# facebookresearch/NasRec

Hardware: AMD Instinct MI355X
Metric: supernet samples/sec at batch 256 (Criteo-shape), 1/2/4/8 MI355X (higher is better)
Workload: dtype f32

## Files before the change

### include/nasrec_hip.h

```cpp
#ifndef NASREC_HIP_H
#define NASREC_HIP_H

#include <stdint.h>

#ifdef __cplusplus
extern "C" {
#endif

#define NASREC_MAX_SEGS 8
#define NASREC_MAX_TABLES 32
#define NASREC_EMB_DIM 16
#define NASREC_MHA_PARAMS 1696
#define NASREC_MHA_SAVED 36

enum {
  NASREC_AM_KC = 0,
  NASREC_AM_RC = 1,
  NASREC_AM_TOKR = 2,
  NASREC_AM_TOKK = 3
};
enum { NASREC_CM_PLAIN = 0,
       NASREC_CM_TOKJ = 1    };
enum { NASREC_ACT_NONE = 0, NASREC_ACT_RELU = 1, NASREC_ACT_SILU = 2, NASREC_ACT_SIGMOID = 3 };

// ... 591 lines not shown
int nasrec_graph_destroy(void* graph);

int nasrec_gemm(void* stream, const nasrec_gemm_desc_t* d);
int nasrec_embedding_gather(void* stream, const nasrec_embed_desc_t* d);
int nasrec_embedding_dedup(void* stream, const nasrec_emb_dedup_desc_t* d);
int nasrec_dot_tri(void* stream, const nasrec_dot_tri_desc_t* d);
int nasrec_fm(void* stream, const nasrec_fm_desc_t* d);
int nasrec_mha_ffn(void* stream, const nasrec_mha_desc_t* d);
int nasrec_layernorm(void* stream, const nasrec_layernorm_desc_t* d);
int nasrec_final_logit(void* stream, const nasrec_final_desc_t* d);
int nasrec_bce_logits(void* stream, const nasrec_bce_desc_t* d);
int nasrec_adagrad_dense(void* stream, const nasrec_adagrad_dense_desc_t* d);
int nasrec_adagrad_rows(void* stream, const nasrec_adagrad_rows_desc_t* d);
int nasrec_opt_reduce(void* stream, const nasrec_opt_reduce_desc_t* d);
int nasrec_opt_apply(void* stream, const nasrec_opt_apply_desc_t* d);
int nasrec_dedup_ids(void* stream, const nasrec_dedup_ids_desc_t* d);
int nasrec_opt_reduce2(void* stream, const nasrec_opt_reduce2_desc_t* d);
int nasrec_final_fused(void* stream, const nasrec_final_desc_t* d);
int nasrec_weight_decay(void* stream, const nasrec_weight_decay_desc_t* d);
int nasrec_opt_moments(void* stream, const nasrec_opt_moments_desc_t* d);
int nasrec_last_layer_step(void* stream, const nasrec_last_layer_step_desc_t* d);
int nasrec_roc_auc(void* stream, const nasrec_roc_auc_desc_t* d);
int64_t nasrec_roc_auc_workspace_bytes(int64_t n);
int nasrec_worklist(void* stream, const nasrec_worklist_desc_t* d);

enum {
  NASREC_GEMM_ROUTE_GENERAL = 0,
  NASREC_GEMM_ROUTE_KSLICE = 1,
  NASREC_GEMM_ROUTE_SKINNY_N = 2,
  NASREC_GEMM_ROUTE_TINYK = 3,
  NASREC_GEMM_ROUTE_TOKEN_LINEAR = 4,
  NASREC_GEMM_ROUTE_TOKEN_DW = 5,
  NASREC_GEMM_ROUTE_FAST = 6,
  NASREC_GEMM_ROUTE_BAD_NSEG = -1,
  NASREC_GEMM_ROUTE_BAD_BINDING = -2,
  NASREC_GEMM_ROUTE_BAD_BALANCED = -3
};
int nasrec_gemm_route(const nasrec_gemm_desc_t* d, unsigned* eligible_mask);

int nasrec_alloc_uncached(int64_t bytes, void** out);
int nasrec_free_uncached(void* p);

int nasrec_event_create(void** ev);
int nasrec_event_record(void* ev, void* stream);
int nasrec_event_elapsed_ms(void* start, void* stop, float* ms);
int nasrec_event_destroy(void* ev);

enum { NASREC_TSV_OK = 0, NASREC_TSV_NEEDS_PYTHON = 1, NASREC_TSV_BAD_COLUMNS = 2 };
int64_t nasrec_tsv_parse(const char* buf, int64_t len, int32_t Fd, int32_t Fs, const int64_t* table_rows, int64_t max_rows,
                         int64_t* label, int64_t* dense, int64_t* cat, int64_t* consumed, int32_t* status);

const char* nasrec_last_error(void);
int nasrec_abi_version(void);
int nasrec_desc_sizes(int32_t* out, int n);

#ifdef __cplusplus
}
#endif
#endif
```

### nasrec_amd/_lib.py

```python
import ctypes as C
import os

import torch

_HERE = os.path.dirname(os.path.abspath(__file__))
LIB_PATH = os.environ.get("NASREC_HIP_LIB") or os.path.join(_HERE, "lib", "libnasrec_hip.so")

MAX_SEGS = 8
MAX_TABLES = 32
EMB_DIM = 16
MHA_PARAMS = 1696
MHA_SAVED = 36
REDUCE_MAX_DST = 48

AM_KC, AM_RC, AM_TOKR, AM_TOKK = 0, 1, 2, 3
CM_PLAIN, CM_TOKJ = 0, 1
ACT_NONE, ACT_RELU, ACT_SILU, ACT_SIGMOID = 0, 1, 2, 3
TSV_OK, TSV_NEEDS_PYTHON, TSV_BAD_COLUMNS = 0, 1, 2
ACT_BY_NAME = {"identity": ACT_NONE, "relu": ACT_RELU, "silu": ACT_SILU}

(OP_GEMM, OP_EMBED_GATHER, OP_DOT_TRI_FWD, OP_DOT_TRI_BWD, OP_FM_FWD, OP_FM_BWD, OP_MHA_FWD, OP_MHA_BWD, OP_REDUCE_ROWS,
 OP_COPY_SEGS, OP_GATE_BWD, OP_ROWSUM, OP_FINAL_FWD, OP_BCE, OP_FINAL_BWD, OP_EMB_DEDUP, OP_SUMSQ, OP_CLIP_COEF,
 OP_ADAGRAD_DENSE, OP_ADAGRAD_ROWS, OP_MEMSET, OP_LAYERNORM_FWD, OP_LAYERNORM_BWD, OP_ADD_SEGS, OP_SCALE,
 OP_ACT_BWD, OP_STAGE_INPUTS, OP_OPT_REDUCE, OP_OPT_APPLY, OP_WORKLIST, OP_CONST_I64, OP_SPLITK_EPILOGUES, OP_DEDUP_IDS,
# ... 84 lines not shown
                ("dlogits_out", vp), ("nsplit", i32), ("dseg_done", i32), ("tok_stride", i32 * MAX_SEGS)]


class BceDesc(C.Structure):
    _fields_ = [("kind", i32), ("B", i32), ("grad_scale", f32), ("_pad", i32), ("logits", vp), ("y", vp), ("loss", vp),
                ("dlogits", vp)]


class SumsqDesc(C.Structure):
    _fields_ = [("kind", i32), ("nblocks", i32), ("n", i64), ("x", vp), ("partial", vp), ("chunks", vp), ("nchunks", i64)]


class ClipCoefDesc(C.Structure):
    _fields_ = [("kind", i32), ("n_a", i32), ("n_b", i32), ("max_norm", f32), ("partial_a", vp), ("partial_b", vp), ("out", vp)]


class AdagradDenseDesc(C.Structure):
    _fields_ = [("kind", i32), ("eps", f32), ("n", i64), ("p", vp), ("g", vp), ("state", vp), ("lr", vp), ("coef", vp),
                ("chunks", vp), ("nchunks", i64)]


class AdagradRowsDesc(C.Structure):
    _fields_ = [("kind", i32), ("B", i32), ("Fs", i32), ("eps", f32), ("idx", vp), ("leader", vp), ("gsum", vp),
                ("table", vp * MAX_TABLES), ("state", vp * MAX_TABLES), ("lr", vp), ("coef", vp), ("rows", i64 * MAX_TABLES),
                ("rank_B", i32), ("_pad", i32), ("rank_stride", i64)]


class MemsetDesc(C.Structure):
    _fields_ = [("kind", i32), ("_pad", i32), ("bytes", i64), ("ptr", vp), ("chunks", vp), ("nchunks", i64)]


SPLITK_BALANCED = -1
(GEMM_ROUTE_GENERAL, GEMM_ROUTE_KSLICE, GEMM_ROUTE_SKINNY_N, GEMM_ROUTE_TINYK, GEMM_ROUTE_TOKEN_LINEAR, GEMM_ROUTE_TOKEN_DW,
 GEMM_ROUTE_FAST) = range(7)
GEMM_ROUTE_BAD_NSEG, GEMM_ROUTE_BAD_BINDING, GEMM_ROUTE_BAD_BALANCED = -1, -2, -3
SK_WORKSPACE_FLOATS = 512 * 3 * 128 * 128
CHUNK_ELEMS = 65536
CONST_I64_MAX = 448


class ConstI64Desc(C.Structure):
    _fields_ = [("kind", i32), ("n", i32), ("dst", vp), ("vals", i64 * CONST_I64_MAX)]


class LayerNormDesc(C.Structure):
    _fields_ = [("kind", i32), ("mode", i32), ("R", i32), ("D", i32), ("ldx", i32), ("ldy", i32), ("act", i32),
                ("dims_in_use", i32), ("accumulate", i32), ("eps", f32), ("x", vp), ("w", vp), ("b", vp), ("y", vp), ("stats", vp),
                ("dy", vp), ("dx", vp), ("dwb_partial", vp), ("nblk", i32), ("_pad", i32)]


class ScaleDesc(C.Structure):
    _fields_ = [("kind", i32), ("_pad", i32), ("n", i64), ("s", f32), ("_pad2", i32), ("x", vp), ("y", vp)]


class ActBwdDesc(C.Structure):
    _fields_ = [("kind", i32), ("mode", i32), ("R", i32), ("D", i32), ("ld_dy", i32), ("ld_z", i32), ("ld_dz", i32), ("act", i32),
                ("dims_in_use", i32), ("dy", vp), ("z", vp), ("dz", vp)]


DEDUP_IDS_MAX_B = 2048


class DedupIdsDesc(C.Structure):
    _fields_ = [("kind", i32), ("B", i32), ("Fs", i32), ("cap", i32), ("idx", vp), ("leader", vp), ("order", vp), ("lists", vp), ("counts", vp),
                ("heads", vp)]


# ... 167 lines not shown
```

### nasrec_amd/csrc/gemm.hip

```cpp
#include "gemm_tile.h"
#include "gemm_ring.h"

template <int AM, int BMODE, int CM, int NT, int TK, int TBM, int TBN>
__global__ __launch_bounds__(NT) void gemm_kernel(const nasrec_gemm_desc_t d, int Mmax, int Nmax) {
  gemm_tile<AM, BMODE, CM, NT, TK, TBM, TBN>(d, Mmax, Nmax, blockIdx.x, blockIdx.y, blockIdx.z);
}

#ifndef GEMM_RING
#define GEMM_RING 4
#endif
template <int AM, int BMODE, int CM, int NT, int TK, int TBM, int TBN, bool AUX>
__global__ __launch_bounds__(NT) void gemm_ring_kernel(const nasrec_gemm_desc_t d, int Mmax, int Nmax) {
  gemm_tile_ring<AM, BMODE, CM, NT, TK, TBM, TBN, AUX, AUX ? 2 : GEMM_RING>(d, Mmax, Nmax, blockIdx.x, blockIdx.y, blockIdx.z);
}

template <int CM>
__global__ __launch_bounds__(256) void gemm_splitk_epilogue(const nasrec_gemm_desc_t d, int Mmax, int Nmax) {
  splitk_second_pass<CM>(d, Mmax, Nmax, blockIdx.z, (long)blockIdx.x * 256 + threadIdx.x);
}

struct EpiGeom {
  int first[NASREC_EPILOGUES_MAX + 1];
  int per[NASREC_EPILOGUES_MAX];
  int Mmax[NASREC_EPILOGUES_MAX], Nmax[NASREC_EPILOGUES_MAX];
// ... 74 lines not shown
    } else if (deep) {
      launch_ring<AM, BMODE, CM, GEMM_MID_NT, GEMM_TK_DEEP, 64, 64>(st, d, Mmax, Nmax, zdim);
    } else {
      launch_ring<AM, BMODE, CM, GEMM_MID_NT, 32, 64, 64>(st, d, Mmax, Nmax, zdim);
    }
  } else if (Nmax >= Mmax) {
    if (deep) launch_ring<AM, BMODE, CM, 256, GEMM_TK_DEEP, 64, 16>(st, d, Mmax, Nmax, zdim);
    else launch_ring<AM, BMODE, CM, 256, 32, 64, 16>(st, d, Mmax, Nmax, zdim);
  } else {
    if (deep) launch_ring<AM, BMODE, CM, 256, GEMM_TK_DEEP, 16, 64>(st, d, Mmax, Nmax, zdim);
    else launch_ring<AM, BMODE, CM, 256, 32, 16, 64>(st, d, Mmax, Nmax, zdim);
  }
}

static constexpr int binding_key(int am, int bm, int cm) { return am * 100 + bm * 10 + cm; }

int nasrec_gemm_route(const nasrec_gemm_desc_t* d, unsigned* eligible_mask) {
  if (eligible_mask) *eligible_mask = 0;
  if (d->nseg < 1 || d->nseg > NASREC_MAX_SEGS) return NASREC_GEMM_ROUTE_BAD_NSEG;
  switch (binding_key(d->amode, d->bmode, d->cmode)) {
    case binding_key(NASREC_AM_KC, NASREC_AM_KC, NASREC_CM_PLAIN):
    case binding_key(NASREC_AM_KC, NASREC_AM_RC, NASREC_CM_PLAIN):
    case binding_key(NASREC_AM_RC, NASREC_AM_RC, NASREC_CM_PLAIN):
    case binding_key(NASREC_AM_KC, NASREC_AM_TOKR, NASREC_CM_TOKJ):
    case binding_key(NASREC_AM_RC, NASREC_AM_TOKR, NASREC_CM_TOKJ):
    case binding_key(NASREC_AM_TOKK, NASREC_AM_TOKK, NASREC_CM_PLAIN):
      break;
    default:
      return NASREC_GEMM_ROUTE_BAD_BINDING;
  }
  static const struct { int family; bool (*takes)(const nasrec_gemm_desc_t*); } ladder[] = {
    {NASREC_GEMM_ROUTE_TOKEN_LINEAR, token_linear_eligible},
    {NASREC_GEMM_ROUTE_KSLICE, gemm_kslice_eligible},
    {NASREC_GEMM_ROUTE_SKINNY_N, gemm_skinny_n_eligible},
    {NASREC_GEMM_ROUTE_TINYK, gemm_tinyk_eligible},
    {NASREC_GEMM_ROUTE_TOKEN_DW, token_dw_eligible},
    {NASREC_GEMM_ROUTE_FAST, gemm_fast_eligible},
  };
  const bool balanced = d->splitk == NASREC_SPLITK_BALANCED;
  int route = balanced ? NASREC_GEMM_ROUTE_BAD_BALANCED : NASREC_GEMM_ROUTE_GENERAL;
  unsigned mask = balanced ? 0u : 1u << NASREC_GEMM_ROUTE_GENERAL;
  bool taken = false;
  for (const auto& f : ladder) {
    if (!f.takes(d)) continue;
    mask |= 1u << f.family;
    if (!taken) route = f.family;
    taken = true;
    if (!eligible_mask) break;
  }
  if (eligible_mask) *eligible_mask = mask;
  return route;
}

int launch_gemm(hipStream_t st, const nasrec_gemm_desc_t* d) {
  const int route = nasrec_gemm_route(d, nullptr);
  if (route == NASREC_GEMM_ROUTE_BAD_NSEG) return nasrec_set_error(-2, "gemm: nseg=%d out of range", d->nseg);
  if (route == NASREC_GEMM_ROUTE_BAD_BINDING)
    return nasrec_set_error(-2, "gemm: unsupported operand binding a=%d b=%d c=%d", d->amode, d->bmode, d->cmode);
  int Mmax = 0, Nmax = 0;
  const int nprob = d->zmode ? d->nseg : 1;
  for (int q = 0; q < nprob; ++q) {
    if (d->seg[q].M > Mmax) Mmax = d->seg[q].M;
    if (d->seg[q].N > Nmax) Nmax = d->seg[q].N;
  }
  if (Mmax <= 0 || Nmax <= 0) return 0;
  const int S = d->splitk > 1 ? d->splitk : 1;
  if (S > 1 && d->workspace == nullptr) return nasrec_set_error(-3, "gemm: splitk=%d needs a workspace", S);
  switch (route) {
    case NASREC_GEMM_ROUTE_TOKEN_LINEAR: return launch_token_linear(st, d);
    case NASREC_GEMM_ROUTE_KSLICE: return launch_gemm_kslice(st, d);
    case NASREC_GEMM_ROUTE_SKINNY_N: return launch_gemm_skinny_n(st, d);
    case NASREC_GEMM_ROUTE_TINYK: return launch_gemm_tinyk(st, d);
    case NASREC_GEMM_ROUTE_BAD_BALANCED:
      return nasrec_set_error(-2, "gemm: the balanced schedule exists for throughput-regime launches only (the planner asks nasrec_gemm_route)");
    case NASREC_GEMM_ROUTE_TOKEN_DW: launch_token_dw(st, d, Mmax, Nmax); break;
    case NASREC_GEMM_ROUTE_FAST: {
      const int rc = launch_gemm_fast(st, d, Mmax, Nmax, nprob * S);
      if (rc) return rc;
      break;
    }
    default:
      switch (binding_key(d->amode, d->bmode, d->cmode)) {
        case binding_key(NASREC_AM_KC, NASREC_AM_KC, NASREC_CM_PLAIN): launch_general_t<NASREC_AM_KC, NASREC_AM_KC, NASREC_CM_PLAIN>(st, d, Mmax, Nmax, nprob, S); break;
        case binding_key(NASREC_AM_KC, NASREC_AM_RC, NASREC_CM_PLAIN): launch_general_t<NASREC_AM_KC, NASREC_AM_RC, NASREC_CM_PLAIN>(st, d, Mmax, Nmax, nprob, S); break;
        case binding_key(NASREC_AM_RC, NASREC_AM_RC, NASREC_CM_PLAIN): launch_general_t<NASREC_AM_RC, NASREC_AM_RC, NASREC_CM_PLAIN>(st, d, Mmax, Nmax, nprob, S); break;
        case binding_key(NASREC_AM_KC, NASREC_AM_TOKR, NASREC_CM_TOKJ): launch_general_t<NASREC_AM_KC, NASREC_AM_TOKR, NASREC_CM_TOKJ>(st, d, Mmax, Nmax, nprob, S); break;
        case binding_key(NASREC_AM_RC, NASREC_AM_TOKR, NASREC_CM_TOKJ): launch_general_t<NASREC_AM_RC, NASREC_AM_TOKR, NASREC_CM_TOKJ>(st, d, Mmax, Nmax, nprob, S); break;
        default: launch_general_t<NASREC_AM_TOKK, NASREC_AM_TOKK, NASREC_CM_PLAIN>(st, d, Mmax, Nmax, nprob, S); break;
      }
  }
  if (S > 1 && !d->defer_second_pass) {
    const dim3 g2((unsigned)(((long)Mmax * Nmax + 255) / 256), 1, nprob);
    if (d->cmode == NASREC_CM_PLAIN) hipLaunchKernelGGL((gemm_splitk_epilogue<NASREC_CM_PLAIN>), g2, dim3(256), 0, st, *d, Mmax, Nmax);
    else hipLaunchKernelGGL((gemm_splitk_epilogue<NASREC_CM_TOKJ>), g2, dim3(256), 0, st, *d, Mmax, Nmax);
  }
  return nasrec_check_launch("gemm");
}
```

### nasrec_amd/csrc/gemm_tile.h

```cpp
#pragma once
#include "common.h"

#ifndef GEMM_TK_DEEP
#define GEMM_TK_DEEP 64
#endif
#ifndef GEMM_XCD_REMAP
#define GEMM_XCD_REMAP 0
#endif
#ifndef GEMM_ZBATCH_TILE32
#define GEMM_ZBATCH_TILE32 1
#endif
#ifndef GEMM_BIG_NT
#define GEMM_BIG_NT 256
#endif
#ifndef GEMM_BIG_TK
#define GEMM_BIG_TK 32
#endif
#ifndef GEMM_MID_NT
#define GEMM_MID_NT 1024
#endif
#ifndef GEMM_SKINNY_BELOW
#define GEMM_SKINNY_BELOW 128
#endif
#ifndef NASREC_GEMM_FAST_MIN_TILES
#define NASREC_GEMM_FAST_MIN_TILES 120
#endif
bool gemm_fast_eligible(const nasrec_gemm_desc_t* d);
int launch_gemm_fast(hipStream_t st, const nasrec_gemm_desc_t* d, int Mmax, int Nmax, int zdim);
bool gemm_kslice_eligible(const nasrec_gemm_desc_t* d);
int launch_gemm_kslice(hipStream_t st, const nasrec_gemm_desc_t* d);
bool gemm_skinny_n_eligible(const nasrec_gemm_desc_t* d);
int launch_gemm_skinny_n(hipStream_t st, const nasrec_gemm_desc_t* d);
bool gemm_tinyk_eligible(const nasrec_gemm_desc_t* d);
int launch_gemm_tinyk(hipStream_t st, const nasrec_gemm_desc_t* d);
bool token_linear_eligible(const nasrec_gemm_desc_t* d);
int launch_token_linear(hipStream_t st, const nasrec_gemm_desc_t* d);
bool token_dw_eligible(const nasrec_gemm_desc_t* d);
int launch_token_dw(hipStream_t st, const nasrec_gemm_desc_t* d, int Mmax, int Nmax);

template <int MODE, int NT, int TK, int R>
__device__ __forceinline__ void stage_coords(int tid, int it, int& rr, int& kk) {
  if (MODE == NASREC_AM_KC || MODE == NASREC_AM_TOKK) {
    kk = tid & (TK - 1);
    rr = tid / TK + (NT / TK) * it;
  } else {
    rr = tid & (R - 1);
    kk = tid / R + (NT / R) * it;
  }
}

__device__ __forceinline__ float mul_lookup(const nasrec_gemm_desc_t& d, int i, int j) {
  for (int q = 0; q < d.mul_nseg; ++q) {
    int jj = j - d.mul_off[q];
    if (jj >= 0 && jj < d.mul_width[q]) return d.mul_ptr[q] ? d.mul_ptr[q][(long)i * d.mul_ld[q] + jj] : 0.f;
  }
  return 0.f;
}

__device__ __forceinline__ int seg_ld(const nasrec_gemm_desc_t& d, int sq, int which) {
  return which ? d.seg[sq].ldb : d.seg[sq].lda;
}

template <int CM>
// ... 397 lines not shown
```

### nasrec_amd/csrc/worklist.hip

```cpp
#include <stdlib.h>
#include <string.h>

#include <vector>

#include "worklist_body.h"

static int wl_gemm_geometry(const nasrec_gemm_desc_t* g, nasrec_wl_item_t& it, int blob_left) {
  if (g->nseg < 1 || g->nseg > NASREC_MAX_SEGS) return nasrec_set_error(-2, "worklist: gemm nseg=%d", g->nseg);
  const int need = (int)offsetof(nasrec_gemm_desc_t, seg) + g->nseg * (int)sizeof(nasrec_gemm_seg_t);
  if (need > blob_left) return nasrec_set_error(-2, "worklist: truncated gemm descriptor (%d bytes) runs past the blob", need);
  const int nprob = g->zmode ? g->nseg : 1;
  const int S = g->splitk > 1 ? g->splitk : 1;
  if (g->splitk == NASREC_SPLITK_BALANCED) return nasrec_set_error(-2, "worklist: the balanced schedule is a throughput-regime launch");
  if ((it.part == 0) != (S == 1)) return nasrec_set_error(-2, "worklist: gemm part %d with splitk %d", it.part, g->splitk);
  if (S > 1 && !g->workspace) return nasrec_set_error(-3, "worklist: splitk=%d needs a workspace", S);
  int Mmax = 0, Nmax = 0, Kmax = 0;
  long wgs = 0;
  bool aux = false, uniform = true;
  for (int q = 0; q < nprob; ++q) {
    Mmax = g->seg[q].M > Mmax ? g->seg[q].M : Mmax;
    Nmax = g->seg[q].N > Nmax ? g->seg[q].N : Nmax;
    wgs += (long)((g->seg[q].M + 63) / 64) * ((g->seg[q].N + 63) / 64) * S;
  }
  for (int q = 0; q < g->nseg; ++q) {
    const nasrec_gemm_seg_t& s = g->seg[q];
    if (s.A && s.K > Kmax) Kmax = s.K;
    aux = aux || s.Aaux || s.Baux;
    if (!g->zmode && (s.ones_col != g->seg[0].ones_col || s.Mvalid != g->seg[0].Mvalid)) uniform = false;
    if (!g->zmode && s.A && ((s.Aaux != nullptr) != (g->seg[0].Aaux != nullptr) || (s.Baux != nullptr) != (g->seg[0].Baux != nullptr))) uniform = false;
  }
  if (!uniform) return nasrec_set_error(-2, "worklist: k-segments that disagree on row predicates / mask operands take the plain template");
  {
    const bool kca = g->amode == NASREC_AM_KC || g->amode == NASREC_AM_TOKK, kcb = g->bmode == NASREC_AM_KC || g->bmode == NASREC_AM_TOKK;
    if (!kca && kcb) return nasrec_set_error(-2, "worklist: operand binding a=%d b=%d has no body", g->amode, g->bmode);
  }
  if (Mmax <= 0 || Nmax <= 0) {
    it.nblk = 0;
    return 0;
  }
  if (it.part == 2) {
    const int per = (int)(((long)Mmax * Nmax + 255) / 256);
    it.geom[0] = per;
    it.nblk = per * nprob;
    return 0;
  }
  static const bool dense_body = getenv("NASREC_WL_DENSE_BODY") == nullptr || atoi(getenv("NASREC_WL_DENSE_BODY")) != 0;
  if (dense_body && it.part == 0 && !g->zmode && !aux && g->amode == NASREC_AM_KC && g->bmode == NASREC_AM_KC && g->cmode == NASREC_CM_PLAIN) {
    bool plain = true;
    int steps = 0;
    for (int q = 0; q < g->nseg; ++q) {
      const nasrec_gemm_seg_t& s = g->seg[q];
      plain = plain && !s.ones_col && !(s.Mvalid > 0 && s.Mvalid < Mmax);
      plain = plain && (long)Mmax * s.lda + s.K < (1L << 29) && (long)Nmax * s.ldb + s.K < (1L << 29);
      steps += (s.A && s.K > 0) ? (s.K + 15) >> 4 : 1;
    }
    if (plain && steps <= 2 * WL_DENSE_STEPS && (Mmax + 15) / 16 < 0x10000) {
      it.geom[0] = (Nmax + 15) / 16;
      it.geom[1] = (Mmax + 15) / 16 | (((steps + WL_DENSE_STEPS - 1) / WL_DENSE_STEPS) << 16);
      it.geom[2] = WL_TOKS | (3 << 2);
      it.nblk = (it.geom[0] * ((Mmax + 15) / 16) + 3) / 4;
      return 0;
    }
  }
  bool aux_b = false;
  for (int q = 0; q < g->nseg; ++q) aux_b = aux_b || g->seg[q].Baux;
  if (dense_body && it.part == 0 && g->zmode && !aux_b && g->amode == NASREC_AM_KC && g->bmode == NASREC_AM_RC && g->cmode == NASREC_CM_PLAIN) {
    bool plain = true;
    int TU = 0;
    for (int q = 0; q < g->nseg; ++q) {
      const nasrec_gemm_seg_t& s = g->seg[q];
      plain = plain && !s.ones_col && !(s.Mvalid > 0 && s.Mvalid < s.M) && s.K <= 16 * WL_DENSE_STEPS && s.M > 0 && s.N > 0;
      plain = plain && (long)s.M * s.lda + s.K < (1L << 29) && (long)s.K * s.ldb + s.N < (1L << 29);
      TU += ((s.M + 15) / 16) * ((s.N + 15) / 16);
    }
    if (plain && TU > 0) {
      it.geom[0] = TU;
      it.geom[1] = 0;
      it.geom[2] = WL_TOKS | (3 << 2);
// ... 224 lines not shown
  out->_pad = 0;
  out->dev = reinterpret_cast<const nasrec_worklist_desc_t*>(dev_buf);
  return 0;
}

int launch_worklist_dev(hipStream_t st, const nasrec_worklist_dev_desc_t* d) {
  if (!d->dev) return nasrec_set_error(-2, "worklist (device-resident): not prepared");
  if (d->total_blocks < 1) return 0;
  const unsigned* pf = d->pf;
  const unsigned* pm = d->pm;
  if (d->big) {
    hipLaunchKernelGGL(worklist_dev_kernel<true>, dim3((unsigned)d->total_blocks), dim3(256), sizeof(float) * WL_LDS_BIG_FLOATS, st, pf[0], pf[1], pf[2], pf[3],
                       pf[4], pf[5], pm[0], pm[1], pm[2], pm[3], pm[4], pm[5], d->dev);
  } else {
    hipLaunchKernelGGL(worklist_dev_kernel<false>, dim3((unsigned)d->total_blocks), dim3(256), sizeof(float) * WL_LDS_FLOATS, st, pf[0], pf[1], pf[2], pf[3],
                       pf[4], pf[5], pm[0], pm[1], pm[2], pm[3], pm[4], pm[5], d->dev);
  }
  return nasrec_check_launch("worklist (device-resident)");
}

#define PS_SPIN_BUDGET_TICKS 1000000ull

template <bool BIG>
__device__ __forceinline__ void ps_run_item(int it_kind, int it_part, int g0, int g1, int g2, unsigned long long blob, int vb, int nblk, int nwg) {
  float* lds = wl_lds;
  const int tid = threadIdx.x, wave = tid >> 6, lane = tid & 63;
  switch (it_kind) {
    case NASREC_OP_GEMM: {
      if (it_part == 2) {
        for (int u = vb; u < nblk; u += nwg) wl_gemm_second_pass(blob, u, g0);
        break;
      }
      const int cfg = g2;
      if ((cfg & 3) == WL_TOKS && ((cfg >> 2) & 3) == 3 && g1 == 0) wl_dense_small_dx(blob, vb, g0);
      else if ((cfg & 3) == WL_TOKS && ((cfg >> 2) & 3) == 3) wl_dense_small(blob, vb, g0, g1);
      else if ((cfg & 3) == WL_TOKS && ((cfg >> 2) & 3) == 1) wl_token_fwd(blob, vb, g0);
      else if ((cfg & 3) == WL_TOKS) wl_token_dx(blob, vb, g0);
      else if ((cfg >> 4) & 1) {
        for (int u = vb; u < nblk; u += nwg) {
          wl_gemm_bind<true>((cfg >> 2) & 3, cfg & 3, blob, u, g0, g1);
          if (u + nwg < nblk) __syncthreads();
        }
      } else {
        for (int u = vb; u < nblk; u += nwg) {
          wl_gemm_bind<false>((cfg >> 2) & 3, cfg & 3, blob, u, g0, g1);
          if (u + nwg < nblk) __syncthreads();
        }
      }
      break;
    }
    case NASREC_OP_MHA_FWD:
      wl_mha_fwd(blob, vb);
      break;
    case NASREC_OP_MHA_BWD:
      if (BIG) mha_bwd_tok(wl_ref<nasrec_mha_desc_t>(blob), __builtin_amdgcn_readfirstlane(vb), wl_lds);
      break;
    case NASREC_OP_FM_FWD: {
      const nasrec_fm_desc_t& d = wl_ref<nasrec_fm_desc_t>(blob);
      const int b = vb * 4 + wave;
      if (b < d.B) fm_fwd_sample(d, b, lane);
      break;
    }
    case NASREC_OP_FM_BWD: {
      const nasrec_fm_desc_t& d = wl_ref<nasrec_fm_desc_t>(blob);
      const int b = vb * 4 + wave;
      if (b < d.B) fm_bwd_sample(d, b, lane);
      break;
// ... 201 lines not shown
```

### nasrec_amd/csrc/worklist_body.h

```cpp
#pragma once
#include "attention_tok.h"
#include "gemm_rt.h"
#include "final_bodies.h"
#include "interact_bodies.h"
#include "dedup_bodies.h"

#define WL_LDS_BIG_FLOATS 9888
#define WL_LDS_FLOATS 7840
static_assert(MHA_TOK_BWD_LDS_FLOATS <= WL_LDS_BIG_FLOATS && MHA_TOK_FWD_LDS_FLOATS <= WL_LDS_FLOATS, "Transformer bodies fit the worklist launches");

#define WL_TK 64
#ifndef WL_AUX_RING2
#define WL_AUX_RING2 0
#endif
enum { WL_TOKS = 0, WL_T32x32 = 1, WL_T64x16 = 2, WL_T16x64 = 3 };

extern __shared__ __attribute__((aligned(16))) float wl_lds[];

template <typename T>
__device__ __forceinline__ const T& wl_ref(unsigned long long addr) {
  const unsigned lo = __builtin_amdgcn_readfirstlane((unsigned)addr), hi = __builtin_amdgcn_readfirstlane((unsigned)(addr >> 32));
  return *(const T*)(const __attribute__((address_space(4))) T*)(((unsigned long long)hi << 32) | lo);
}

// ... 142 lines not shown
    fk += 16;
    const bool next = fk >= K;
    fq = next ? fq + 1 : fq;
    fk = next ? 0 : fk;
  }
  if (batch == 0 && g.bias) {
    const float warm = g.bias[g.bias_on_rows ? row : col];
    asm volatile("" ::"v"(warm));
  }
#pragma unroll
  for (int slot = 0; slot < WL_DENSE_STEPS; ++slot) {
    const int l = lim[slot];
    if (l > 0) {
      f32x4 a = fa[slot], b = fb[slot];
      if (l < 16) {
#pragma unroll
        for (int j = 0; j < 4; ++j) {
          const bool in = 4 * fg + j < l;
          a[j] = in ? a[j] : 0.f;
          b[j] = in ? b[j] : 0.f;
        }
      }
#pragma unroll
      for (int j = 0; j < 4; ++j) acc = __builtin_amdgcn_mfma_f32_16x16x4f32(a[j], b[j], acc, 0, 0, 0);
    }
  }
  }
  {
    const float v4[4] = {acc[0], acc[1], acc[2], acc[3]};
    if (mt * 16 + 4 * fg < M && nt * 16 + e < N) epilogue_store_col4<NASREC_CM_PLAIN>(g, s0, mt * 16 + 4 * fg, nt * 16 + e, M, v4);
  }
}

__device__ __forceinline__ void wl_dense_small_dx(unsigned long long blob, int vb_, int TU_) {
  const nasrec_gemm_desc_t& g = wl_ref<nasrec_gemm_desc_t>(blob);
  const int vb = __builtin_amdgcn_readfirstlane(vb_), TU = __builtin_amdgcn_readfirstlane(TU_);
  const int lane = threadIdx.x & 63, wave = __builtin_amdgcn_readfirstlane(threadIdx.x >> 6);
  const int e = lane & 15, fg = lane >> 4;
  wl_warm_blob(blob, (int)offsetof(nasrec_gemm_desc_t, seg) + g.nseg * (int)sizeof(nasrec_gemm_seg_t));
  int t = vb * 4 + wave, q = 0;
  if (t >= TU) return;
  while (q < g.nseg - 1 && t >= ((g.seg[q].M + 15) >> 4) * ((g.seg[q].N + 15) >> 4)) t -= ((g.seg[q].M + 15) >> 4) * ((g.seg[q].N + 15) >> 4), ++q;
  const nasrec_gemm_seg_t& sg = g.seg[q];
  const int M = sg.M, N = sg.N, K = sg.K, NT = (N + 15) >> 4;
  const int mt = t / NT, nt = t - mt * NT;
  if (!sg.A || K <= 0) {
    if (!sg.accumulate) {
#pragma unroll
      for (int r = 0; r < 4; ++r) {
        const int i = mt * 16 + 4 * fg + r, j = nt * 16 + e;
        if (i < M && j < N) epilogue_store<NASREC_CM_PLAIN>(g, sg, i, j, 0.f);
      }
    }
    return;
  }
  const int row = min(mt * 16 + e, M - 1), col = min(nt * 16 + e, N - 1);
  const __amdgpu_buffer_rsrc_t ra = __builtin_amdgcn_make_buffer_rsrc(const_cast<float*>(sg.A), 0, (int)(4 * ((long)(M - 1) * sg.lda + K)), 0x00020000);
  const float* wp = sg.B + col;
  f32x4 fa[WL_DENSE_STEPS];
  float fb[WL_DENSE_STEPS][4];
#pragma unroll
  for (int s = 0; s < WL_DENSE_STEPS; ++s) {
    fa[s] = __builtin_bit_cast(f32x4, __builtin_amdgcn_raw_buffer_load_b128(ra, 4 * (row * sg.lda + 16 * s + 4 * fg), 0, 0));
#pragma unroll
    for (int j = 0; j < 4; ++j) fb[s][j] = wp[(long)min(16 * s + 4 * fg + j, K - 1) * sg.ldb];
  }
// ... 125 lines not shown
  if (f01 != WL_PACKED_NONE) {
    const unsigned f[6] = {f01, f23, f45, f67, f89, fab}, m[6] = {m01, m23, m45, m67, m89, mab};
    unsigned meta = m01 & 0xffffu;
#pragma unroll
    for (int q = 1; q < NASREC_WL_MAX_ITEMS; ++q) {
      const unsigned fq = (f[q >> 1] >> (16 * (q & 1))) & 0xffffu, mq = (m[q >> 1] >> (16 * (q & 1))) & 0xffffu;
      if ((unsigned)bid >= fq) {
        k = q;
        it_first = (int)fq;
        meta = mq;
      }
    }
    it_kind = meta & 63;
    it_part = (meta >> 6) & 3;
    it_off = (int)(meta >> 8) * 16;
  } else {
#pragma unroll 1
    while (k + 1 < wl.n && bid >= wl.item[k + 1].first) ++k;
    it_first = wl.item[k].first;
    it_kind = wl.item[k].kind;
    it_part = wl.item[k].part;
    it_off = wl.item[k].off;
  }
  const nasrec_wl_item_t& it = wl.item[k];
  const int vb = bid - it_first;
  const unsigned long long blob = base + offsetof(nasrec_worklist_desc_t, blob) + it_off;
  switch (it_kind) {
    case NASREC_OP_GEMM: {
      if (it_part == 2) {
        wl_gemm_second_pass(blob, vb, it.geom[0]);
        break;
      }
      const int cfg = it.geom[2];
      if ((cfg & 3) == WL_TOKS && ((cfg >> 2) & 3) == 3 && it.geom[1] == 0) wl_dense_small_dx(blob, vb, it.geom[0]);
      else if ((cfg & 3) == WL_TOKS && ((cfg >> 2) & 3) == 3) wl_dense_small(blob, vb, it.geom[0], it.geom[1]);
      else if ((cfg & 3) == WL_TOKS && ((cfg >> 2) & 3) == 1) wl_token_fwd(blob, vb, it.geom[0]);
      else if ((cfg & 3) == WL_TOKS) wl_token_dx(blob, vb, it.geom[0]);
      else if ((cfg >> 4) & 1) wl_gemm_bind<true>((cfg >> 2) & 3, cfg & 3, blob, vb, it.geom[0], it.geom[1]);
      else wl_gemm_bind<false>((cfg >> 2) & 3, cfg & 3, blob, vb, it.geom[0], it.geom[1]);
      break;
    }
    case NASREC_OP_MHA_FWD:
      wl_mha_fwd(blob, vb);
      break;
    case NASREC_OP_MHA_BWD:
      if (BIG) mha_bwd_tok(wl_ref<nasrec_mha_desc_t>(blob), __builtin_amdgcn_readfirstlane(vb), wl_lds);
      break;
    case NASREC_OP_FM_FWD: {
      const nasrec_fm_desc_t& d = wl_ref<nasrec_fm_desc_t>(blob);
      const int b = vb * 4 + wave;
      if (b < d.B) fm_fwd_sample(d, b, lane);
      break;
    }
    case NASREC_OP_FM_BWD: {
      const nasrec_fm_desc_t& d = wl_ref<nasrec_fm_desc_t>(blob);
      const int b = vb * 4 + wave;
      if (b < d.B) fm_bwd_sample(d, b, lane);
      break;
    }
    case NASREC_OP_DOT_TRI_FWD: {
      const nasrec_dot_tri_desc_t& d = wl_ref<nasrec_dot_tri_desc_t>(blob);
      const int b = vb * 4 + wave;
      if (b < d.B) dot_tri_fwd_sample(d, b, lane, lds + wave * (d.k1 * TRI_LD));
      break;
    }
    case NASREC_OP_DOT_TRI_BWD: {
      const nasrec_dot_tri_desc_t& d = wl_ref<nasrec_dot_tri_desc_t>(blob);
// ... 50 lines not shown
```

### nasrec_amd/plan.py

```python
import ctypes as C
import math
from typing import Dict, List, Optional

import torch

from . import _lib as L

NUM_MHA_HEADS = 8
DS_INTERACT_NUM_SPLITS = 8
E = 16

DENSE_UNARY = ("linear-2d", "zeros-2d")
DENSE_BINARY = ("sum", "sigmoid-gating")
DENSE_SPARSE = ("dot-product",)
SPARSE_NODES = ("zeros-3d", "transformer", "linear-3d")

MHA_LEAVES = ["_mha.in_proj_weight", "_mha.in_proj_bias", "_mha.out_proj.weight", "_mha.out_proj.bias", "_attn_ln.weight",
              "_attn_ln.bias", "attn_fc1.weight", "attn_fc1.bias", "attn_fc2.weight", "attn_fc2.bias", "_attn_fc_ln.weight",
              "_attn_fc_ln.bias"]
MHA_SHAPES = [(48, 16), (48,), (16, 16), (16,), (16,), (16,), (16, 16), (16,), (16, 16), (16,), (16,), (16,)]
MHA_OFFS = [0, 768, 816, 1072, 1088, 1104, 1120, 1376, 1392, 1648, 1664, 1680]


class NetConfig:
# ... 269 lines not shown
        d = L.ConstI64Desc()
        d.kind = L.OP_CONST_I64
        d.n = len(part)
        d.dst = dst_ptr + 8 * i
        d.vals[:len(part)] = part
        out.append(d)
    return out


import os as _os
_SPLITK_CAP = int(_os.environ["NASREC_SPLITK_CAP"]) if _os.environ.get("NASREC_SPLITK_CAP") else None


def _splitk_for(tiles_mn, ktiles, nprob=1):
    if tiles_mn * nprob >= 192 or ktiles < 8:
        return 1
    if _SPLITK_CAP is not None:
        return max(1, min(_SPLITK_CAP, ktiles // 2, max(1, 256 // max(1, tiles_mn * nprob))))
    s = min(ktiles // 2, max(1, 256 // max(1, tiles_mn * nprob)))
    return max(1, min(s, 32))


_LN_NBLK = int(_os.environ.get("NASREC_LN_NBLK", "512"))
_TOKDW_CAP = int(_os.environ.get("NASREC_TOKDW_CAP", "128"))
_FAST_MIN_KT = int(_os.environ.get("NASREC_FAST_MIN_KT", "4"))


def gemm_route(d):
    mask = C.c_uint()
    return L.load().nasrec_gemm_route(C.addressof(d), C.byref(mask)), mask.value


_KSLICE_BIT, _SKINNY_N_BIT, _FAST_BIT = 1 << L.GEMM_ROUTE_KSLICE, 1 << L.GEMM_ROUTE_SKINNY_N, 1 << L.GEMM_ROUTE_FAST


def _fast_gemm_splitk(d, tiles, kt, mask1):
    if tiles <= 0:
        return None
    S = 1
    if tiles < 256:
        S = max(1, min(-(-256 // tiles), kt // _FAST_MIN_KT, 32))
    if S > 1:
        d.splitk = S
        mask1 = gemm_route(d)[1]
        d.splitk = 1
    return S if mask1 & _FAST_BIT else None


BALANCED_MIN_SAVING_US = float(_os.environ.get("NASREC_BALANCED_MIN_US", "80.0"))


def _balanced_schedule_pays(segs, zmode):
    live = [sd for sd in segs if sd.get("A")]
    if not live or len(live) != len(segs):
        return False
    if zmode:
        kts = {(sd["K"] + 31) // 32 for sd in segs}
        if len(kts) != 1:
            return False
        T = kts.pop()
        probs = segs
    else:
        T = sum((sd["K"] + 31) // 32 for sd in segs)
        probs = segs[:1]
    tiles = sum(((sd["M"] + 127) // 128) * ((sd["N"] + 127) // 128) for sd in probs)
    left = tiles % 512
    if left == 0:
        return False
    rounds = tiles // 512 + (1.0 if left > 64 else 0.55)
    return (rounds - tiles / 512.0) * T * 3.8 >= BALANCED_MIN_SAVING_US


_ROUTE_KERNEL = {L.GEMM_ROUTE_GENERAL: "gemm_kernel", L.GEMM_ROUTE_KSLICE: "gemm_kslice_kernel", L.GEMM_ROUTE_SKINNY_N: "gemm_skinny_n_kernel",
                 L.GEMM_ROUTE_TINYK: "gemm_tinyk_kernel", L.GEMM_ROUTE_TOKEN_LINEAR: "token_linear_kernel",
                 L.GEMM_ROUTE_TOKEN_DW: "token_dw_kernel", L.GEMM_ROUTE_FAST: "gemm_fast_kernel"}


def gemm_kernel_name(d) -> str:
    family = gemm_route(d)[0]
    if family < 0:
        raise ValueError("nasrec_gemm rejects this descriptor (nasrec_gemm_route: %d)" % family)
    return _ROUTE_KERNEL[family]


def gemm_descs(ctx, amode, bmode, cmode, segs, zmode, act=0, bias_on_rows=0, mask_on_rows=0, dims=-1, beta=0, bias=None, save_z=None,
               save_act=None, pre_add=None, mul=None, splitk=None, rowsum_out=None):
    if not segs:
        return []
    nseg = len(segs)
    assert nseg <= L.MAX_SEGS
    d = L.GemmDesc()
    d.kind = L.OP_GEMM
    d.amode, d.bmode, d.cmode = amode, bmode, cmode
    d.nseg = nseg
    d.zmode = zmode
    if act:
        d.act = act
    if bias_on_rows:
        d.bias_on_rows = bias_on_rows
    if mask_on_rows:
        d.mask_on_rows = mask_on_rows
    d.dims_in_use = dims
    if beta:
        d.beta = beta
    if bias:
        d.bias = bias
    if save_z:
        d.save_z = save_z
# ... 25 lines not shown
        kt = (sdict["K"] + 31) // 32
        kt_sum += kt
        if kt > kt_max:
            kt_max = kt
        if sdict.get("A"):
            fast_kt_sum += kt
            if kt > fast_kt_max:
                fast_kt_max = kt
        if zmode or q == 0:
            fast_tiles += ((m + 127) // 128) * ((n + 127) // 128)
        live_tiles += ((m + 63) // 64) * ((n + 63) // 64)
    B = ctx.B
    if zmode:
        S = _splitk_for(live_tiles, kt_max)
    else:
        S = _splitk_for(((M + 63) // 64) * ((N + 63) // 64), kt_sum)
    d.splitk = 1
    mask1 = gemm_route(d)[1]
    fast = _fast_gemm_splitk(d, fast_tiles, fast_kt_max if zmode else fast_kt_sum, mask1) if B > 128 else None
    if fast is not None:
        S = fast
    if amode == L.AM_TOKK and zmode and B >= 1024:
        ok = True
        for sd in segs:
            if sd["M"] > 80 or sd["N"] > 80 or sd.get("Aaux") or sd.get("Baux"):
                ok = False
                break
        if ok:
            S = max(4, min(_TOKDW_CAP, 256 // nseg, B // 64))
    if splitk is not None:
        S = splitk
    elif B <= 512 and S > 1 and mask1 & _KSLICE_BIT:
        S = 1
    elif B >= 1024 and mask1 & _SKINNY_N_BIT:
        S = 1
    if fast == 1 and S == 1 and B > 256 and ctx.sk_workspace is not None and _balanced_schedule_pays(segs, zmode):
        d.splitk = L.SPLITK_BALANCED
        d.workspace = ctx.sk_workspace().data_ptr()
    if S > 1:
        d.splitk = S
        ws = ctx.alloc(S * M * N * (nseg if zmode else 1))
        d.workspace = ws.data_ptr()
    if rowsum_out is not None:
        d.rowsum_out = rowsum_out
    return [d]


def _live_segs(segs: List[Seg]):
    return [s for s in segs if s.view is not None]


def _cover_pieces(live: List[Seg]):
    cuts = sorted({s.koff for s in live} | {s.koff + s.width for s in live})
    out = []
    for a, b in zip(cuts[:-1], cuts[1:]):
        rank = 0
        for s in live:
            if s.koff <= a and b <= s.koff + s.width:
                if out and out[-1][0] is s and out[-1][2] == a and out[-1][3] == rank:
                    out[-1] = (s, out[-1][1], b, rank)
                else:
                    out.append((s, a, b, rank))
                rank += 1
    return out


# ... 980 lines not shown
```

Baseline: 1.161 million.

## Add deep-K GEMM route splitting K across waves with LDS reduction

```diff
diff --git a/include/nasrec_hip.h b/include/nasrec_hip.h
--- a/include/nasrec_hip.h
+++ b/include/nasrec_hip.h
@@ -647,6 +647,7 @@
   NASREC_GEMM_ROUTE_TOKEN_LINEAR = 4,
   NASREC_GEMM_ROUTE_TOKEN_DW = 5,
   NASREC_GEMM_ROUTE_FAST = 6,
+  NASREC_GEMM_ROUTE_DEEPK = 7,
   NASREC_GEMM_ROUTE_BAD_NSEG = -1,
   NASREC_GEMM_ROUTE_BAD_BINDING = -2,
   NASREC_GEMM_ROUTE_BAD_BALANCED = -3
diff --git a/nasrec_amd/_lib.py b/nasrec_amd/_lib.py
--- a/nasrec_amd/_lib.py
+++ b/nasrec_amd/_lib.py
@@ -140,7 +140,7 @@
 
 SPLITK_BALANCED = -1
 (GEMM_ROUTE_GENERAL, GEMM_ROUTE_KSLICE, GEMM_ROUTE_SKINNY_N, GEMM_ROUTE_TINYK, GEMM_ROUTE_TOKEN_LINEAR, GEMM_ROUTE_TOKEN_DW,
- GEMM_ROUTE_FAST) = range(7)
+ GEMM_ROUTE_FAST, GEMM_ROUTE_DEEPK) = range(8)
 GEMM_ROUTE_BAD_NSEG, GEMM_ROUTE_BAD_BINDING, GEMM_ROUTE_BAD_BALANCED = -1, -2, -3
 SK_WORKSPACE_FLOATS = 512 * 3 * 128 * 128
 CHUNK_ELEMS = 65536
diff --git a/nasrec_amd/csrc/gemm.hip b/nasrec_amd/csrc/gemm.hip
--- a/nasrec_amd/csrc/gemm.hip
+++ b/nasrec_amd/csrc/gemm.hip
@@ -130,6 +130,7 @@
   static const struct { int family; bool (*takes)(const nasrec_gemm_desc_t*); } ladder[] = {
     {NASREC_GEMM_ROUTE_TOKEN_LINEAR, token_linear_eligible},
     {NASREC_GEMM_ROUTE_KSLICE, gemm_kslice_eligible},
+    {NASREC_GEMM_ROUTE_DEEPK, gemm_deepk_eligible},
     {NASREC_GEMM_ROUTE_SKINNY_N, gemm_skinny_n_eligible},
     {NASREC_GEMM_ROUTE_TINYK, gemm_tinyk_eligible},
     {NASREC_GEMM_ROUTE_TOKEN_DW, token_dw_eligible},
@@ -167,6 +168,7 @@
   switch (route) {
     case NASREC_GEMM_ROUTE_TOKEN_LINEAR: return launch_token_linear(st, d);
     case NASREC_GEMM_ROUTE_KSLICE: return launch_gemm_kslice(st, d);
+    case NASREC_GEMM_ROUTE_DEEPK: return launch_gemm_deepk(st, d);
     case NASREC_GEMM_ROUTE_SKINNY_N: return launch_gemm_skinny_n(st, d);
     case NASREC_GEMM_ROUTE_TINYK: return launch_gemm_tinyk(st, d);
     case NASREC_GEMM_ROUTE_BAD_BALANCED:
diff --git a/nasrec_amd/csrc/gemm_tile.h b/nasrec_amd/csrc/gemm_tile.h
--- a/nasrec_amd/csrc/gemm_tile.h
+++ b/nasrec_amd/csrc/gemm_tile.h
@@ -29,6 +29,8 @@
 int launch_gemm_fast(hipStream_t st, const nasrec_gemm_desc_t* d, int Mmax, int Nmax, int zdim);
 bool gemm_kslice_eligible(const nasrec_gemm_desc_t* d);
 int launch_gemm_kslice(hipStream_t st, const nasrec_gemm_desc_t* d);
+bool gemm_deepk_eligible(const nasrec_gemm_desc_t* d);
+int launch_gemm_deepk(hipStream_t st, const nasrec_gemm_desc_t* d);
 bool gemm_skinny_n_eligible(const nasrec_gemm_desc_t* d);
 int launch_gemm_skinny_n(hipStream_t st, const nasrec_gemm_desc_t* d);
 bool gemm_tinyk_eligible(const nasrec_gemm_desc_t* d);
diff --git a/nasrec_amd/csrc/worklist.hip b/nasrec_amd/csrc/worklist.hip
--- a/nasrec_amd/csrc/worklist.hip
+++ b/nasrec_amd/csrc/worklist.hip
@@ -4,6 +4,35 @@
 #include <vector>
 
 #include "worklist_body.h"
+
+static int deepk_steps(const nasrec_gemm_desc_t* d) {
+  long steps = 0;
+  for (int q = 0; q < d->nseg; ++q) steps += (d->seg[q].A && d->seg[q].K > 0) ? ((long)d->seg[q].K + 15) >> 4 : 1;
+  return steps > 0x7fffffffL ? 0x7fffffff : (int)steps;
+}
+
+bool gemm_deepk_eligible(const nasrec_gemm_desc_t* d) {
+  if (d->amode != NASREC_AM_KC || d->bmode != NASREC_AM_KC || d->cmode != NASREC_CM_PLAIN || d->zmode || d->splitk > 1 || d->splitk < 0) return false;
+  const nasrec_gemm_seg_t& s0 = d->seg[0];
+  if (s0.M < 1 || s0.M > 512 || s0.N < 1) return false;
+  for (int q = 0; q < d->nseg; ++q) {
+    const nasrec_gemm_seg_t& s = d->seg[q];
+    if (s.Aaux || s.Baux || s.ones_col || (s.Mvalid > 0 && s.Mvalid < s0.M)) return false;
+    if (s.A && s.K > 0 && ((long)s0.M * s.lda + s.K >= (1L << 29) || (long)s0.N * s.ldb + s.K >= (1L << 29))) return false;
+  }
+  const long tiles = (long)((s0.M + 15) / 16) * ((s0.N + 15) / 16);
+  return tiles <= WL_DEEPK_MAX_TILES && deepk_steps(d) > 2 * WL_DENSE_STEPS;
+}
+
+__global__ __launch_bounds__(256, 4) void gemm_deepk_kernel(const nasrec_gemm_desc_t d, int NT, int T) {
+  wl_deepk((unsigned long long)__builtin_amdgcn_kernarg_segment_ptr(), blockIdx.x, NT, T);
+}
+
+int launch_gemm_deepk(hipStream_t st, const nasrec_gemm_desc_t* d) {
+  const int MT = (d->seg[0].M + 15) / 16, NT = (d->seg[0].N + 15) / 16;
+  hipLaunchKernelGGL(gemm_deepk_kernel, dim3((unsigned)(MT * NT)), dim3(256), sizeof(float) * WL_DEEPK_LDS_FLOATS, st, *d, NT, deepk_steps(d));
+  return nasrec_check_launch("gemm_deepk");
+}
 
 static int wl_gemm_geometry(const nasrec_gemm_desc_t* g, nasrec_wl_item_t& it, int blob_left) {
   if (g->nseg < 1 || g->nseg > NASREC_MAX_SEGS) return nasrec_set_error(-2, "worklist: gemm nseg=%d", g->nseg);
@@ -44,6 +73,13 @@
     it.nblk = per * nprob;
     return 0;
   }
+  if (it.part == 0 && nasrec_gemm_route(g, nullptr) == NASREC_GEMM_ROUTE_DEEPK) {
+    it.geom[0] = (Nmax + 15) / 16;
+    it.geom[1] = deepk_steps(g);
+    it.geom[2] = WL_DEEPK_CFG;
+    it.nblk = it.geom[0] * ((Mmax + 15) / 16);
+    return 0;
+  }
   static const bool dense_body = getenv("NASREC_WL_DENSE_BODY") == nullptr || atoi(getenv("NASREC_WL_DENSE_BODY")) != 0;
   if (dense_body && it.part == 0 && !g->zmode && !aux && g->amode == NASREC_AM_KC && g->bmode == NASREC_AM_KC && g->cmode == NASREC_CM_PLAIN) {
     bool plain = true;
@@ -334,7 +370,8 @@
         break;
       }
       const int cfg = g2;
-      if ((cfg & 3) == WL_TOKS && ((cfg >> 2) & 3) == 3 && g1 == 0) wl_dense_small_dx(blob, vb, g0);
+      if (cfg == WL_DEEPK_CFG) wl_deepk(blob, vb, g0, g1);
+      else if ((cfg & 3) == WL_TOKS && ((cfg >> 2) & 3) == 3 && g1 == 0) wl_dense_small_dx(blob, vb, g0);
       else if ((cfg & 3) == WL_TOKS && ((cfg >> 2) & 3) == 3) wl_dense_small(blob, vb, g0, g1);
       else if ((cfg & 3) == WL_TOKS && ((cfg >> 2) & 3) == 1) wl_token_fwd(blob, vb, g0);
       else if ((cfg & 3) == WL_TOKS) wl_token_dx(blob, vb, g0);
diff --git a/nasrec_amd/csrc/worklist_body.h b/nasrec_amd/csrc/worklist_body.h
--- a/nasrec_amd/csrc/worklist_body.h
+++ b/nasrec_amd/csrc/worklist_body.h
@@ -198,6 +198,95 @@
   }
 }
 
+#define WL_DEEPK_MAX_TILES 256
+#define WL_DEEPK_CFG (WL_TOKS | (3 << 2) | (1 << 5))
+#define WL_DEEPK_LDS_FLOATS (3 * 64 * 4)
+__device__ __forceinline__ void wl_deepk(unsigned long long blob, int vb_, int NT_, int T_) {
+  const nasrec_gemm_desc_t& g = wl_ref<nasrec_gemm_desc_t>(blob);
+  const int vb = __builtin_amdgcn_readfirstlane(vb_), NT = __builtin_amdgcn_readfirstlane(NT_), T = __builtin_amdgcn_readfirstlane(T_);
+  const int lane = threadIdx.x & 63, wave = __builtin_amdgcn_readfirstlane(threadIdx.x >> 6);
+  const int e = lane & 15, fg = lane >> 4;
+  wl_warm_blob(blob, (int)offsetof(nasrec_gemm_desc_t, seg) + g.nseg * (int)sizeof(nasrec_gemm_seg_t));
+  const nasrec_gemm_seg_t& s0 = g.seg[0];
+  const int M = s0.M, N = s0.N;
+  const int mt = vb / NT, nt = vb - mt * NT;
+  const int row = min(mt * 16 + e, M - 1), col = min(nt * 16 + e, N - 1);
+  const int t0 = (wave * T) >> 2;
+  int left = (((wave + 1) * T) >> 2) - t0;
+  const int mine = left;
+  int fq = 0, fk = 0;
+  for (int t = t0; fq < g.nseg; ++fq) {
+    const int n = (g.seg[fq].A && g.seg[fq].K > 0) ? (g.seg[fq].K + 15) >> 4 : 1;
+    if (t < n) {
+      fk = 16 * t;
+      break;
+    }
+    t -= n;
+  }
+  f32x4 fa[WL_DENSE_STEPS], fb[WL_DENSE_STEPS];
+  int lim[WL_DENSE_STEPS];
+  f32x4 acc0 = {0.f, 0.f, 0.f, 0.f}, acc1 = {0.f, 0.f, 0.f, 0.f};
+  auto fetch = [&](int slot) {
+    const bool in = left > 0 && fq < g.nseg;
+    const nasrec_gemm_seg_t& sg = g.seg[in ? fq : 0];
+    const bool live = in && sg.A != nullptr && sg.K > 0;
+    const int K = live ? sg.K : 0, kk = fk + 4 * fg;
+    lim[slot] = K - fk;
+    const __amdgpu_buffer_rsrc_t ra =
+        __builtin_amdgcn_make_buffer_rsrc(const_cast<float*>(sg.A), 0, live ? (int)(4 * ((long)(M - 1) * sg.lda + K)) : 0, 0x00020000);
+    const __amdgpu_buffer_rsrc_t rb =
+        __builtin_amdgcn_make_buffer_rsrc(const_cast<float*>(sg.B), 0, live ? (int)(4 * ((long)(N - 1) * sg.ldb + K)) : 0, 0x00020000);
+    fa[slot] = __builtin_bit_cast(f32x4, __builtin_amdgcn_raw_buffer_load_b128(ra, 4 * (row * sg.lda + kk), 0, 0));
+    fb[slot] = __builtin_bit_cast(f32x4, __builtin_amdgcn_raw_buffer_load_b128(rb, 4 * (col * sg.ldb + kk), 0, 0));
+    left -= 1;
+    fk += 16;
+    const bool next = fk >= K;
+    fq = next ? fq + 1 : fq;
+    fk = next ? 0 : fk;
+  };
+  auto multiply = [&](int slot, f32x4& acc) {
+    const int l = lim[slot];
+    if (l <= 0) return;
+    f32x4 a = fa[slot], b = fb[slot];
+    if (l < 16) {
+#pragma unroll
+      for (int j = 0; j < 4; ++j) {
+        const bool in = 4 * fg + j < l;
+        a[j] = in ? a[j] : 0.f;
+        b[j] = in ? b[j] : 0.f;
+      }
+    }
+#pragma unroll
+    for (int j = 0; j < 4; ++j) acc = __builtin_amdgcn_mfma_f32_16x16x4f32(a[j], b[j], acc, 0, 0, 0);
+  };
+#pragma unroll
+  for (int slot = 0; slot < WL_DENSE_STEPS; ++slot) fetch(slot);
+  if (wave == 0 && g.bias) {
+    const float warm = g.bias[g.bias_on_rows ? row : col];
+    asm volatile("" ::"v"(warm));
+  }
+  for (int t = 0; t < mine; t += WL_DENSE_STEPS) {
+#pragma unroll
+    for (int slot = 0; slot < WL_DENSE_STEPS; ++slot) {
+      multiply(slot, (slot & 1) ? acc1 : acc0);
+      fetch(slot);
+    }
+  }
+  f32x4 acc = acc0 + acc1;
+  if (wave) *reinterpret_cast<f32x4*>(&wl_lds[((wave - 1) * 64 + lane) * 4]) = acc;
+  __syncthreads();
+  if (wave) return;
+  {
+    const f32x4 q1 = *reinterpret_cast<const f32x4*>(&wl_lds[(0 * 64 + lane) * 4]), q2 = *reinterpret_cast<const f32x4*>(&wl_lds[(1 * 64 + lane) * 4]),
+                q3 = *reinterpret_cast<const f32x4*>(&wl_lds[(2 * 64 + lane) * 4]);
+    acc = (acc + q1) + (q2 + q3);
+  }
+  {
+    const float v4[4] = {acc[0], acc[1], acc[2], acc[3]};
+    if (mt * 16 + 4 * fg < M && nt * 16 + e < N) epilogue_store_col4<NASREC_CM_PLAIN>(g, s0, mt * 16 + 4 * fg, nt * 16 + e, M, v4);
+  }
+}
+
 __device__ __forceinline__ void wl_dense_small_dx(unsigned long long blob, int vb_, int TU_) {
   const nasrec_gemm_desc_t& g = wl_ref<nasrec_gemm_desc_t>(blob);
   const int vb = __builtin_amdgcn_readfirstlane(vb_), TU = __builtin_amdgcn_readfirstlane(TU_);
@@ -389,7 +478,8 @@
         break;
       }
       const int cfg = it.geom[2];
-      if ((cfg & 3) == WL_TOKS && ((cfg >> 2) & 3) == 3 && it.geom[1] == 0) wl_dense_small_dx(blob, vb, it.geom[0]);
+      if (cfg == WL_DEEPK_CFG) wl_deepk(blob, vb, it.geom[0], it.geom[1]);
+      else if ((cfg & 3) == WL_TOKS && ((cfg >> 2) & 3) == 3 && it.geom[1] == 0) wl_dense_small_dx(blob, vb, it.geom[0]);
       else if ((cfg & 3) == WL_TOKS && ((cfg >> 2) & 3) == 3) wl_dense_small(blob, vb, it.geom[0], it.geom[1]);
       else if ((cfg & 3) == WL_TOKS && ((cfg >> 2) & 3) == 1) wl_token_fwd(blob, vb, it.geom[0]);
       else if ((cfg & 3) == WL_TOKS) wl_token_dx(blob, vb, it.geom[0]);
diff --git a/nasrec_amd/plan.py b/nasrec_amd/plan.py
--- a/nasrec_amd/plan.py
+++ b/nasrec_amd/plan.py
@@ -325,6 +325,7 @@
 
 
 _KSLICE_BIT, _SKINNY_N_BIT, _FAST_BIT = 1 << L.GEMM_ROUTE_KSLICE, 1 << L.GEMM_ROUTE_SKINNY_N, 1 << L.GEMM_ROUTE_FAST
+_DEEPK_BIT = 1 << L.GEMM_ROUTE_DEEPK
 
 
 def _fast_gemm_splitk(d, tiles, kt, mask1):
@@ -366,7 +367,7 @@
 
 _ROUTE_KERNEL = {L.GEMM_ROUTE_GENERAL: "gemm_kernel", L.GEMM_ROUTE_KSLICE: "gemm_kslice_kernel", L.GEMM_ROUTE_SKINNY_N: "gemm_skinny_n_kernel",
                  L.GEMM_ROUTE_TINYK: "gemm_tinyk_kernel", L.GEMM_ROUTE_TOKEN_LINEAR: "token_linear_kernel",
-                 L.GEMM_ROUTE_TOKEN_DW: "token_dw_kernel", L.GEMM_ROUTE_FAST: "gemm_fast_kernel"}
+                 L.GEMM_ROUTE_TOKEN_DW: "token_dw_kernel", L.GEMM_ROUTE_FAST: "gemm_fast_kernel", L.GEMM_ROUTE_DEEPK: "gemm_deepk_kernel"}
 
 
 def gemm_kernel_name(d) -> str:
@@ -458,6 +459,8 @@
         S = splitk
     elif B <= 512 and S > 1 and mask1 & _KSLICE_BIT:
         S = 1
+    elif B <= 512 and S > 1 and mask1 & _DEEPK_BIT:
+        S = 1
     elif B >= 1024 and mask1 & _SKINNY_N_BIT:
         S = 1
     if fast == 1 and S == 1 and B > 256 and ctx.sk_workspace is not None and _balanced_schedule_pays(segs, zmode):
```

Result: no change. 1.160 million (-0.1%).
